# changlin31/AutoProg

Measured on AMD Instinct MI355X. Metric: images/sec/GPU (fwd+bwd) VOLO-D1 224px AutoProg step, higher is better.
Workload: dtype bf16; 1 GPU; BASELINE.json configs[1]: volo_h12_l18 (VOLO-D1) 224px token-label training step; model=volo_h12_l18, global_batch=128, per_gpu_batch=128, res=224, parallelism=dp1, step=fwd+loss+bwd+AdamW+4xEMA, deterministic=False

## Files before the change

autoprog_amd/_lib.py:

```python
import ctypes
import os

import torch
from ctypes import POINTER, Structure, c_char_p, c_float, c_int, c_int64, c_void_p

_HERE = os.path.dirname(os.path.abspath(__file__))
LIB_PATH = os.environ.get("AP_LIB_PATH") or os.path.join(_HERE, "libautoprog_hip.so")


class GemmEpilogue(Structure):
    _fields_ = [("bias", c_void_p), ("gelu", c_int), ("preact_out", c_void_p), ("dgelu_of", c_void_p),
                ("row_scale", c_void_p), ("rows_per_scale", c_int), ("residual", c_void_p), ("ldr", c_int), ("mul_by", c_void_p),
                ("mul_by8", c_void_p), ("q8_out", c_void_p), ("q8_scale", c_void_p), ("q8_amax", c_void_p)]


class MlpFusedArgs(Structure):
    _fields_ = [("x", c_void_p), ("ldx", c_int), ("wa", c_void_p), ("ldwa", c_int), ("wb", c_void_p), ("ldwb", c_int), ("out", c_void_p), ("ldo", c_int),
                ("hidden_out", c_void_p), ("ldh", c_int), ("codes", c_void_p), ("bias1", c_void_p), ("bias2", c_void_p),
                ("row_scale_hidden", c_void_p), ("row_scale_out", c_void_p), ("rows_per_scale", c_int), ("residual", c_void_p), ("ldr", c_int),
                ("m", c_int), ("c", c_int), ("hidden", c_int), ("backward", c_int),
                ("ln_in", c_void_p), ("ld_ln", c_int), ("ln_out", c_void_p), ("ld_lno", c_int), ("ln_gamma", c_void_p), ("ln_beta", c_void_p),
                ("ln_eps", c_float), ("ln_mean", c_void_p), ("ln_rstd", c_void_p)]


# ... 99 lines not shown
_SIGNATURES["ap_conv7_s2d_stat_rows"] = (_I, [_I, _I, _I])
_SIGNATURES["ap_conv7_s2d"] = (_I, [_P, _P, _P, _I, _I, _I, _P, _P])
_SIGNATURES["ap_conv7_s2d_wgrad_workspace"] = (ctypes.c_size_t, [_I, _I, _I])
_SIGNATURES["ap_conv7_s2d_wgrad"] = (_I, [_P, _P, _P, _I, _I, _I, _P, ctypes.c_size_t, _P])
_SIGNATURES["ap_layernorm_bwd_partial"] = (_I, [_P, _P, _P, _P, _P, _P, _P, _L, _I, _P, ctypes.c_size_t, POINTER(c_int), _P])
_SIGNATURES["ap_layernorm_bwd_reduce_batched"] = (_I, [_P, _I, _P])
_SIGNATURES["ap_quantize_fp8"] = (_I, [_P, _P, _L, _P, _P, _P])
_SIGNATURES["ap_quantize_fp8_multi"] = (_I, [_P, _I, _P, _P, _P])
_SIGNATURES["ap_quantize_bf8"] = (_I, [_P, _P, _L, _P, _P, _P, _I, _I, _P, _F, _P, _P])
_SIGNATURES["ap_gemm_tn8_grouped_workspace"] = (ctypes.c_size_t, [_P, _I])
_SIGNATURES["ap_gemm_tn8_acc_grouped"] = (_I, [_P, _I, _P, ctypes.c_size_t, _P])
_SIGNATURES["ap_gemm_tn8_acc_grouped_ln"] = (_I, [_P, _I, _P, _I, _P, ctypes.c_size_t, _P])
_SIGNATURES["ap_debug_poison_lds"] = (_I, [ctypes.c_uint, _P, _P])
_SIGNATURES["ap_conv3x3_c64_bn"] = (_I, [_P, POINTER(BnInput), _P, _P, _I, _I, _I, _P, _P])
_SIGNATURES["ap_conv3x3_c64_wgrad_bn"] = (_I, [_P, POINTER(BnInput), _P, _P, _I, _I, _I, _P, ctypes.c_size_t, _P])
_SIGNATURES["ap_conv3x3_c64_bwd_stats"] = (_I, [_P, _P, _P, _I, _I, _I, _P, POINTER(BnInput), _P, _P])
_SIGNATURES["ap_bn_relu_bwd_act"] = (_I, [_P, _P, _P, _P, _P, _P, _P, _P, _P, _P, _L, _I, _P, ctypes.c_size_t, _P])
_SIGNATURES["ap_bn_relu_bwd_partials"] = (_I, [_P, _P, _P, _P, _P, _P, _P, _I, _P, _P, _P, _L, _I, _P, ctypes.c_size_t, _P])
_SIGNATURES["ap_mhsa_fwd_fp8"] = (_I, [_P, _P, _P, _P, _P, _P, _I, _I, _I, _I, _F, _P, _P])
_SIGNATURES["ap_gemm_nt_fp8"] = (_I, [_P, _I, _P, _I, _P, _I, _I, _I, _I, _P, _P, POINTER(GemmEpilogue), _P])
_SIGNATURES["ap_gemm_nt_patch"] = (_I, [_P, _P, _I, _P, _I, _I, _I, _I, _P, POINTER(PatchMap), _I, _P])
_SIGNATURES["ap_gemm_nt_patch_bn"] = (_I, [_P, POINTER(BnInput), _P, _I, _P, _I, _I, _I, _I, _P, POINTER(PatchMap), _I, _P])
_SIGNATURES["ap_bn_relu_fwd_partials"] = (_I, [_P, _P, _I, _P, _P, _P, _P, _F, _F, _P, _P, _P, _L, _I, _P])
_SIGNATURES["ap_conv3x3_c64_stat_rows"] = (_I, [_I, _I, _I])
_SIGNATURES["ap_conv3x3_c64_pack"] = (_I, [_P, _P, _P, _P])
_SIGNATURES["ap_conv3x3_c64"] = (_I, [_P, _P, _P, _I, _I, _I, _P, _P])
_SIGNATURES["ap_conv3x3_c64_wgrad_workspace"] = (ctypes.c_size_t, [_I, _I, _I])
_SIGNATURES["ap_conv3x3_c64_wgrad"] = (_I, [_P, _P, _P, _I, _I, _I, _P, ctypes.c_size_t, _P])
_SIGNATURES["ap_conv7_s2d_ld"] = (_I, [_P, _P, _P, _I, _I, _I, _I, _P, _P])
_SIGNATURES["ap_conv7_s2d_wgrad_ld"] = (_I, [_P, _P, _I, _P, _I, _I, _I, _P, ctypes.c_size_t, _P])
_SIGNATURES["ap_conv3x3_c128_pack"] = (_I, [_P, _P, _P, _P])
_SIGNATURES["ap_conv3x3_c128_stat_rows"] = (_I, [_I, _I, _I])
_SIGNATURES["ap_conv3x3_c128"] = (_I, [_P, _P, _P, _I, _I, _I, _P, _P])
_SIGNATURES["ap_conv3x3_c128_wgrad_workspace"] = (ctypes.c_size_t, [_I, _I, _I])
_SIGNATURES["ap_conv3x3_c128_wgrad"] = (_I, [_P, _P, _P, _I, _I, _I, _P, ctypes.c_size_t, _P])
_SIGNATURES["ap_sum_reps_acc"] = (_I, [_P, _P, _L, _I, _P])

_SIGNATURES["ap_mlp_fused"] = (_I, [POINTER(MlpFusedArgs), _P])
_SIGNATURES["ap_mlp_fused_infer"] = (_I, [POINTER(MlpFusedArgs), _P])
_SIGNATURES["ap_classify_stats"] = (_I, [_P, _I, _I, _P, _P, _P, _L, _P])
_SIGNATURES["ap_input_prep"] = (_I, [POINTER(InputPrepArgs), _P])
_SIGNATURES["ap_calib_copy"] = (_I, [_P, _P, _L, _P])
_SIGNATURES["ap_calib_mfma"] = (_I, [_P, _P, _I, _P])
_SIGNATURES["ap_grad_health_workspace"] = (ctypes.c_size_t, [_L, _I])
_SIGNATURES["ap_grad_health"] = (_I, [_P, _L, _P, _I, _P, _P, _P, _F, _F, _P, ctypes.c_size_t, _P])
_SIGNATURES["ap_adamw_ema_step_guarded"] = (_I, _SIGNATURES["ap_adamw_ema_step"][1][:-1] + [_P, _P])
_SIGNATURES["ap_adamw_ema_step_ema16"] = (_I, _SIGNATURES["ap_adamw_ema_step"][1][:-1] + [POINTER(c_void_p), _P, _P])
_SIGNATURES["ap_softmax_topk_rows"] = (_I, [_P, _I, _I, _I, _F, _P, _P, _L, _L, _I, _L, _P])
_SIGNATURES["ap_distill_fwd_bwd"] = (_I, [_P, _I, _P, _I, _I, _I, _F, _P, _P, _F, _L, _P])
_SIGNATURES["ap_soft_ce_sparse_gt_fwd_bwd"] = (_I, [_P, _I, _P, _P, _I, _L, _L, _L, _F, _P, _P, _F, _L, _I, _F, _I, _P, _P])
_SIGNATURES["ap_crop_resize_u8"] = (_I, [POINTER(CropResizeArgs), _P])
_SIGNATURES["ap_crop_resample_u8"] = (_I, [POINTER(CropResampleArgs), _P])
_SIGNATURES["ap_randaug_u8"] = (_I, [POINTER(RandAugArgs), _P])

EXPORTED_SYMBOLS = tuple(_SIGNATURES.keys())
EXPECTED_ABI = 7


class AutoProgHipError(RuntimeError):
    pass


def _load():
    if not os.path.isfile(LIB_PATH):
        raise AutoProgHipError(
            "libautoprog_hip.so is missing (%s). Build it with `python -c 'import __graft_entry__ as g; g.build()'` "
            "or `make -C autoprog_amd/csrc`; there is no CPU/PyTorch fallback." % LIB_PATH)
    lib = ctypes.CDLL(LIB_PATH)
    lib.ap_abi_version.restype = ctypes.c_int
    got = lib.ap_abi_version()
    if got != EXPECTED_ABI:
        raise AutoProgHipError("%s has ABI version %d, these bindings were written for %d: rebuild it (make -C autoprog_amd/csrc)"
                               % (LIB_PATH, got, EXPECTED_ABI))
    for name, (res, args) in _SIGNATURES.items():
        fn = getattr(lib, name)
        fn.restype = res
        fn.argtypes = args
    return lib


lib = _load()


def check(code, what):
    if code != 0:
        raise AutoProgHipError("%s failed: %s (code %d)" % (what, lib.ap_error_string(code).decode(), code))
```

autoprog_amd/functional.py:

```python
import math

import os

import torch

from . import ops, wgrad
from ._lib import AutoProgHipError

BF16 = torch.bfloat16


class _WeightBank:

    generation = 0

    @classmethod
    def _key(cls, p):
        return (p.data_ptr(), p._version, cls.generation, tuple(p.shape))

    @staticmethod
    def _flat(p):
        w = p.detach()
        return w.reshape(w.shape[0], -1).contiguous()

# ... 444 lines not shown
    if not keep:
        del n2, m2, r2
    c2 = ops.gemm_nt(a, bank.get(fc2_w), bias=fc2_b, residual=c1)
    if not keep:
        return c2
    return c2, (c0, t0, mc, rc, mt, rt, nc, nt, kv_t, kv_c, q, o, probs, c1, m2, r2, n2, h, a)


class ClassBlockFn(torch.autograd.Function):

    @staticmethod
    def forward(ctx, cls, tok, n1w, n1b, kv_w, kv_b, q_w, q_b, proj_w, proj_b, n2w, n2b, fc1_w, fc1_b, fc2_w, fc2_b, B, N, heads, eps):
        params = (n1w, n1b, kv_w, kv_b, q_w, q_b, proj_w, proj_b, n2w, n2b, fc1_w, fc1_b, fc2_w, fc2_b)
        c2, kept = _class_forward(cls, tok, *params, B, N, heads, eps, keep=True)
        ctx.save_for_backward(*kept, *params)
        ctx.cfg = (B, N, heads, (q_w.shape[0] // heads) ** -0.5)
        ctx.shapes = (cls.shape, tok.shape)
        ctx.set_materialize_grads(False)
        return c2, tok

    @staticmethod
    def backward(ctx, dc2, dtok_pass):
        (c0, t0, mc, rc, mt, rt, nc, nt, kv_t, kv_c, q, o, probs, c1, m2, r2, n2, h, a,
         n1w, n1b, kv_w, kv_b, q_w, q_b, proj_w, proj_b, n2w, n2b, fc1_w, fc1_b, fc2_w, fc2_b) = ctx.saved_tensors
        B, N, heads, scale = ctx.cfg
        params = (n1w, n1b, kv_w, kv_b, q_w, q_b, proj_w, proj_b, n2w, n2b, fc1_w, fc1_b, fc2_w, fc2_b)
        bufs, sunk = wgrad._param_grad_buffers(params)
        (dn1w, dn1b, dkv_w, dkv_b, dq_w, dq_b, dproj_w, dproj_b, dn2w, dn2b, dfc1_w, dfc1_b, dfc2_w, dfc2_b) = bufs
        g = dc2.contiguous() if dc2 is not None else torch.zeros(c0.shape, dtype=BF16, device=c0.device)
        dpass = dtok_pass.reshape(t0.shape).contiguous() if dtok_pass is not None else None
        with wgrad.wgrad_batch() as batch:
            dh = _linear_bwd(g, a, fc2_w, dfc2_w, dfc2_b, **_gelu_bwd_kw(h))
            dn2 = _linear_bwd(dh, n2, fc1_w, dfc1_w, dfc1_b)
            dc1 = ops.layernorm_bwd(dn2, c1, n2w, m2, r2, g, dn2w, dn2b, defer=batch.ln)
            do = _linear_bwd(dc1, o, proj_w, dproj_w, dproj_b)
            dq, dkv_t, dkv_c = ops.class_attn_bwd(q, kv_t, probs, do, B, N + 1, heads, scale, kv_cls=kv_c)
            dnt = _linear_bwd(dkv_t, nt, kv_w, dkv_w, dkv_b)
            dnc_kv = _linear_bwd(dkv_c, nc, kv_w, dkv_w, dkv_b)
            _linear_bwd(dq, nc, q_w, dq_w, dq_b, need_dx=False)
            wq_t = bank.get_t(q_w)
            dnc = ops.gemm_nt(dq, wq_t, n=wq_t.shape[0], k=wq_t.shape[1], residual=dnc_kv)
            dcls = ops.layernorm_bwd(dnc, c0, n1w, mc, rc, dc1, dn1w, dn1b)
            dtok = ops.layernorm_bwd(dnt, t0, n1w, mt, rt, dpass, dn1w, dn1b, defer=batch.ln)
        return (dcls.view(ctx.shapes[0]), dtok.view(ctx.shapes[1]), *wgrad._finish_param_grads(params, bufs, sunk, batch.deferred), None, None, None, None)


def class_block(cls, tok, *args):
    if infer_mode():
        return _class_forward(cls, tok, *args, keep=False), tok
    return ClassBlockFn.apply(cls, tok, *args)


FUSE_POOL_BWD = os.environ.get("AP_FUSE_POOL_BWD", "1") != "0"


def _outlooker_forward(x, n1w, n1b, v_w, v_b, attn_w, attn_b, proj_w, proj_b, n2w, n2b, fc1_w, fc1_b, fc2_w, fc2_b, heads, eps, *, keep):
    B, H, W, C = x.shape
    T = B * H * W
    x2 = x.reshape(T, C).contiguous()
    scale = (C // heads) ** -0.5
    xn1, m1, r1 = ops.layernorm_fwd(x2, n1w, n1b, eps)
    v = ops.gemm_nt(xn1, bank.get(v_w), bias=v_b)
    pooled2 = ops.avgpool2_fwd(xn1.view(B, H, W, C)).view(-1, C)
    if not keep:
        del xn1, m1, r1
    logits = ops.gemm_nt(pooled2, bank.get(attn_w), bias=attn_b)
    if not keep:
        del pooled2
    yo = ops.outlook_fwd(v.view(B, H, W, C), logits, heads, scale)
    if not keep:
        del v, logits
    x1 = ops.gemm_nt(yo.view(T, C), bank.get(proj_w), bias=proj_b, residual=x2)
    if not keep:
        del yo, x2
    xn2, m2, r2 = ops.layernorm_fwd(x1, n2w, n2b, eps)
    a, h = _fc1_fwd(xn2, fc1_w, fc1_b, keep)
    if not keep:
        del xn2, m2, r2
    y = ops.gemm_nt(a, bank.get(fc2_w), bias=fc2_b, residual=x1).view(x.shape)
    if not keep:
        return y
    return y, (x2, m1, r1, xn1, v, pooled2, logits, yo, x1, m2, r2, xn2, h, a)


class OutlookerBlockFn(torch.autograd.Function):

    @staticmethod
    def forward(ctx, x, n1w, n1b, v_w, v_b, attn_w, attn_b, proj_w, proj_b, n2w, n2b, fc1_w, fc1_b, fc2_w, fc2_b,
                heads, eps):
        params = (n1w, n1b, v_w, v_b, attn_w, attn_b, proj_w, proj_b, n2w, n2b, fc1_w, fc1_b, fc2_w, fc2_b)
        y, kept = _outlooker_forward(x, *params, heads, eps, keep=True)
        ctx.save_for_backward(*kept, *params)
        B, H, W, C = x.shape
        ctx.cfg = (B, H, W, C, heads, (C // heads) ** -0.5)
        return y

    @staticmethod
    def backward(ctx, dy):
        (x2, m1, r1, xn1, v, pooled2, logits, yo, x1, m2, r2, xn2, h, a,
         n1w, n1b, v_w, v_b, attn_w, attn_b, proj_w, proj_b, n2w, n2b, fc1_w, fc1_b, fc2_w, fc2_b) = ctx.saved_tensors
        B, H, W, C, heads, scale = ctx.cfg
        T = B * H * W
        params = (n1w, n1b, v_w, v_b, attn_w, attn_b, proj_w, proj_b, n2w, n2b, fc1_w, fc1_b, fc2_w, fc2_b)
        bufs, sunk = wgrad._param_grad_buffers(params)
        (dn1w, dn1b, dv_w, dv_b, dattn_w, dattn_b, dproj_w, dproj_b, dn2w, dn2b, dfc1_w, dfc1_b, dfc2_w, dfc2_b) = bufs
        dy2 = dy.reshape(T, C).contiguous()
        with wgrad.wgrad_batch(sunk, params) as batch:
            dh = _linear_bwd(dy2, a, fc2_w, dfc2_w, dfc2_b, **_gelu_bwd_kw(h))
            dxn2 = _linear_bwd(dh, xn2, fc1_w, dfc1_w, dfc1_b)
            dx1 = ops.layernorm_bwd(dxn2, x1, n2w, m2, r2, dy2, dn2w, dn2b, defer=batch.ln)
            dyo = _linear_bwd(dx1, yo.view(T, C), proj_w, dproj_w, dproj_b)
            dv, dlogits = ops.outlook_bwd(v.view(B, H, W, C), logits, dyo.view(B, H, W, C), heads, scale)
            dpooled = _linear_bwd(dlogits, pooled2, attn_w, dattn_w, dattn_b, n=attn_w.shape[0])
            dxn1 = _linear_bwd(dv.view(T, C), xn1, v_w, dv_w, dv_b)
            dx = ops.layernorm_bwd(dxn1, x2, n1w, m1, r1, dx1, dn1w, dn1b, defer=batch.ln, pool=(dpooled.view(B, (H + 1) // 2, (W + 1) // 2, C), (B, H, W))) if FUSE_POOL_BWD else None
            if dx is None:
                ops.avgpool2_bwd_acc(dpooled.view(B, (H + 1) // 2, (W + 1) // 2, C), dxn1.view(B, H, W, C))
                dx = ops.layernorm_bwd(dxn1, x2, n1w, m1, r1, dx1, dn1w, dn1b, defer=batch.ln)
        return (dx.view(dy.shape), *wgrad._finish_param_grads(params, bufs, sunk, batch.deferred), None, None)


def outlooker_block(x, *args):
    if infer_mode():
        return _outlooker_forward(x, *args, keep=False)
    return OutlookerBlockFn.apply(x, *args)


class LayerNormFn(torch.autograd.Function):
# ... 658 lines not shown
```

autoprog_amd/ops.py:

```python
import ctypes
import math
import os
from collections import namedtuple

import torch

from . import _lib
from ._lib import CropResampleArgs, CropResizeArgs, GemmEpilogue, InputPrepArgs, LnReduce, RandAugArgs, TnProblem, LN_MAX_BATCH, PREP_MAX_BOXES, TN_MAX_GROUP, TN_MAX_GROUP_DET, AutoProgHipError, check, lib

BF16 = torch.bfloat16


_raw_stream = getattr(torch._C, "_cuda_getCurrentRawStream", None)
_cur_device = getattr(torch._C, "_cuda_getDevice", None)


def _stream():
    if _raw_stream is not None and _cur_device is not None:
        return _raw_stream(_cur_device())
    return torch.cuda.current_stream().cuda_stream


def _req_fail(t, dtype, name):
    if not (torch.is_tensor(t) and t.is_cuda):
# ... 521 lines not shown
            if csw is not None:
                _req(csw, BF16, "colsum_weight")
                if csw.numel() < round_up(a.shape[0], 8) or csw.data_ptr() % 16:
                    raise AutoProgHipError("colsum_weight needs ceil(M/8)*8 elements and 16-byte alignment")
            q.colsum_weight = csw.data_ptr() if csw is not None else None
            q.colsum_scale = float(css)
        ptr = ctypes.cast(arr, ctypes.c_void_p)
        ws, ws_bytes = None, 0
        if deterministic:
            ws_bytes = lib.ap_gemm_tn_grouped_workspace(ptr, len(chunk))
            ws = torch.empty(max(ws_bytes // 4, 1), dtype=torch.float32, device=chunk[0].a.device)
        if ln:
            check(lib.ap_gemm_tn_acc_grouped_ln(ptr, len(chunk), ctypes.cast(_ln_reduce_array(ln), ctypes.c_void_p), len(ln), ws.data_ptr() if ws is not None else None,
                                                ws_bytes, _stream()), "ap_gemm_tn_acc_grouped_ln")
            ln = []
        else:
            check(lib.ap_gemm_tn_acc_grouped(ptr, len(chunk), ws.data_ptr() if ws is not None else None, ws_bytes, _stream()), "ap_gemm_tn_acc_grouped")


def colsum_acc(a, out, n=None):
    _req(a, BF16, "a"); _req(out, torch.float32, "out")
    n = out.numel() if n is None else n
    check(lib.ap_colsum_acc(a.data_ptr(), a.shape[1], out.data_ptr(), a.shape[0], n, _stream()), "ap_colsum_acc")
    return out


def outlook_fwd(v, logits, heads, scale):
    _req(v, BF16, "v"); _req(logits, BF16, "logits")
    B, H, W, C = v.shape
    y = torch.empty_like(v)
    check(lib.ap_outlook_fwd(v.data_ptr(), logits.data_ptr(), logits.shape[-1], y.data_ptr(), B, H, W, heads, C // heads,
                             float(scale), _stream()), "ap_outlook_fwd")
    return y


def outlook_bwd(v, logits, dy, heads, scale):
    _req(v, BF16, "v"); _req(logits, BF16, "logits"); _req(dy, BF16, "dy")
    B, H, W, C = v.shape
    dv = torch.empty_like(v)
    dlogits = torch.empty_like(logits)
    check(lib.ap_outlook_bwd(v.data_ptr(), logits.data_ptr(), logits.shape[-1], dy.data_ptr(), dv.data_ptr(), dlogits.data_ptr(),
                             B, H, W, heads, C // heads, float(scale), _stream()), "ap_outlook_bwd")
    return dv, dlogits


def avgpool2_fwd(x):
    _req(x, BF16, "x")
    B, H, W, C = x.shape
    y = torch.empty((B, (H + 1) // 2, (W + 1) // 2, C), dtype=BF16, device=x.device)
    check(lib.ap_avgpool2_fwd(x.data_ptr(), y.data_ptr(), B, H, W, C, _stream()), "ap_avgpool2_fwd")
    return y


def avgpool2_bwd_acc(dpooled, dx):
    _req(dpooled, BF16, "dpooled"); _req(dx, BF16, "dx")
    B, H, W, C = dx.shape
    check(lib.ap_avgpool2_bwd_acc(dpooled.data_ptr(), dx.data_ptr(), B, H, W, C, _stream()), "ap_avgpool2_bwd_acc")
    return dx


def mhsa_emits_fp8(N, hd):
    e = os.environ.get("AP_MHSA_FLASH")
    return (e == "1") if e is not None else (N > 256 or hd == 48)


def mhsa_fwd(qkv, B, N, heads, scale, out_row_scale=None, fp8=None):
    _req(qkv, BF16, "qkv")
    C = qkv.shape[-1] // 3
    out = torch.empty((B * N, C), dtype=BF16, device=qkv.device)
    lse = torch.empty((B, heads, N), dtype=torch.float32, device=qkv.device)
    if fp8 is not None:
        out8 = torch.empty((B * N, C), dtype=torch.uint8, device=qkv.device)
        check(lib.ap_mhsa_fwd_fp8(qkv.data_ptr(), out.data_ptr(), out8.data_ptr(), fp8[0].data_ptr(), fp8[1].data_ptr() if fp8[1] is not None else None,
                                  lse.data_ptr(), B, N, heads, C // heads, float(scale),
                                  out_row_scale.data_ptr() if out_row_scale is not None else None, _stream()), "ap_mhsa_fwd_fp8")
        return out, lse, out8
    check(lib.ap_mhsa_fwd(qkv.data_ptr(), out.data_ptr(), lse.data_ptr(), B, N, heads, C // heads, float(scale),
                          out_row_scale.data_ptr() if out_row_scale is not None else None, _stream()), "ap_mhsa_fwd")
    return out, lse


def mhsa_bwd(qkv, out, dout, lse, B, N, heads, scale):
    _req(qkv, BF16, "qkv"); _req(out, BF16, "out"); _req(dout, BF16, "dout")
    C = qkv.shape[-1] // 3
    dqkv = torch.empty_like(qkv)
    ws_bytes = lib.ap_mhsa_bwd_workspace(B, N, heads, C // heads)
    ws = torch.empty(ws_bytes // 4, dtype=torch.float32, device=qkv.device) if ws_bytes else None
    check(lib.ap_mhsa_bwd(qkv.data_ptr(), out.data_ptr(), dout.data_ptr(), lse.data_ptr(), dqkv.data_ptr(), B, N, heads, C // heads,
                          float(scale), ws.data_ptr() if ws is not None else None, ws_bytes, _stream()), "ap_mhsa_bwd")
    return dqkv


def class_attn_fwd(q, kv, B, N, heads, scale, kv_cls=None):
    _req(q, BF16, "q"); _req(kv, BF16, "kv")
    C = q.shape[-1]
    out = torch.empty((B, C), dtype=BF16, device=q.device)
    probs = torch.empty((B, heads, N), dtype=torch.float32, device=q.device)
    check(lib.ap_class_attn_fwd(q.data_ptr(), kv.data_ptr(), kv_cls.data_ptr() if kv_cls is not None else None, out.data_ptr(), probs.data_ptr(),
                                B, N, heads, C // heads, float(scale), _stream()), "ap_class_attn_fwd")
    return out, probs


def class_attn_bwd(q, kv, probs, dout, B, N, heads, scale, kv_cls=None):
    _req(dout, BF16, "dout")
    dq = torch.empty_like(q)
    dkv = torch.empty_like(kv)
# ... 517 lines not shown
```

include/autoprog_hip.h:

```cpp
#ifndef AUTOPROG_HIP_H
#define AUTOPROG_HIP_H

#include <stddef.h>
#include <stdint.h>

#ifdef __cplusplus
extern "C" {
#endif

typedef void* ap_stream_t;
typedef uint16_t ap_bf16;

enum {
    AP_OK = 0,
    AP_ERR_SHAPE = -1,
    AP_ERR_UNSUPPORTED = -2,
    AP_ERR_LAUNCH = -3,
    AP_ERR_NULL = -4
};

#define AP_MAX_ROWS 0x7fffff00

int ap_abi_version(void);
const char* ap_error_string(int code);
// ... 78 lines not shown
int ap_quantize_fp8(const ap_bf16* x, unsigned char* y, int64_t n, const float* scale, float* amax, ap_stream_t stream);
typedef struct ap_fp8_job { const ap_bf16* x; unsigned char* y; int64_t n; int slot; int pad_; } ap_fp8_job;
int ap_quantize_fp8_multi(const ap_fp8_job* jobs_device, int njobs, const float* scales, float* amax, ap_stream_t stream);

int ap_debug_poison_lds(unsigned pattern, unsigned* scratch2, ap_stream_t stream);
int ap_gemm_nt_fp8(const unsigned char* A, int lda, const unsigned char* B, int ldb, ap_bf16* C, int ldc, int M, int N, int K,
                   const float* dq_a, const float* dq_b, const struct ap_gemm_epilogue* epi, ap_stream_t stream);
int ap_gemm_tn_acc(const ap_bf16* A, int lda, const ap_bf16* B, int ldb, float* C, int ldc,
                   int M, int N1, int N2, float* colsum_A, ap_stream_t stream);
#define AP_TN_MAX_GROUP 32
typedef struct ap_tn_problem {
    const ap_bf16* A; int lda;
    const ap_bf16* B; int ldb;
    float* C; int ldc;
    int M, N1, N2;
    float alpha;
    float* colsum_A;
    const ap_bf16* colsum_weight;
    float colsum_scale;
    const struct ap_patch_map* b_patch;
    const struct ap_bn_input* b_bn;
} ap_tn_problem;
size_t ap_gemm_tn_grouped_workspace(const ap_tn_problem* problems, int count);
int ap_gemm_tn_acc_grouped(const ap_tn_problem* problems, int count, void* workspace, size_t ws_bytes, ap_stream_t stream);
int ap_gemm_tn_acc_grouped_ln(const ap_tn_problem* problems, int count, const ap_ln_reduce* ln_items, int ln_count,
                              void* workspace, size_t ws_bytes, ap_stream_t stream);
#define AP_BF8_COLSUM_SPLITS 64
int ap_quantize_bf8(const ap_bf16* g, unsigned char* y, int64_t n, const float* scale, float* amax, float* colsum, int rows, int cols,
                    const ap_bf16* colsum_weight, float colsum_scale, float* colsum_ws, ap_stream_t stream);
#define AP_FP8_E4M3 0
#define AP_FP8_E5M2 1
typedef struct ap_tn8_problem {
    const unsigned char* A; int lda;
    const unsigned char* B; int ldb;
    float* C; int ldc;
    int M, N1, N2;
    int a_fmt;
    float alpha;
    const float* dq_a; const float* dq_b;
} ap_tn8_problem;
size_t ap_gemm_tn8_grouped_workspace(const ap_tn8_problem* problems, int count);
int ap_gemm_tn8_acc_grouped(const ap_tn8_problem* problems, int count, void* workspace, size_t ws_bytes, ap_stream_t stream);
int ap_gemm_tn8_acc_grouped_ln(const ap_tn8_problem* problems, int count, const ap_ln_reduce* ln_items, int ln_count,
                               void* workspace, size_t ws_bytes, ap_stream_t stream);
int ap_colsum_acc(const ap_bf16* A, int lda, float* out, int M, int N, ap_stream_t stream);

int ap_outlook_fwd(const ap_bf16* v, const ap_bf16* logits, int ldl, ap_bf16* y,
                   int B, int H, int W, int heads, int hd, float scale, ap_stream_t stream);
int ap_outlook_bwd(const ap_bf16* v, const ap_bf16* logits, int ldl, const ap_bf16* dy,
                   ap_bf16* dv, ap_bf16* dlogits, int B, int H, int W, int heads, int hd,
                   float scale, ap_stream_t stream);
int ap_avgpool2_fwd(const ap_bf16* x, ap_bf16* y, int B, int H, int W, int C, ap_stream_t stream);
int ap_avgpool2_bwd_acc(const ap_bf16* dpooled, ap_bf16* dx, int B, int H, int W, int C, ap_stream_t stream);

int ap_mhsa_fwd(const ap_bf16* qkv, ap_bf16* out, float* lse, int B, int N, int heads, int hd,
                float scale, const float* out_row_scale, ap_stream_t stream);
int ap_mhsa_fwd_fp8(const ap_bf16* qkv, ap_bf16* out, unsigned char* out8, const float* q_scale, float* q_amax, float* lse, int B, int N,
                    int heads, int hd, float scale, const float* out_row_scale, ap_stream_t stream);
size_t ap_mhsa_bwd_workspace(int B, int N, int heads, int hd);
int ap_mhsa_bwd(const ap_bf16* qkv, const ap_bf16* out, const ap_bf16* dout, const float* lse,
                ap_bf16* dqkv, int B, int N, int heads, int hd, float scale,
                void* workspace, size_t ws_bytes, ap_stream_t stream);

int ap_class_attn_fwd(const ap_bf16* q, const ap_bf16* kv, const ap_bf16* kv_cls , ap_bf16* out, float* probs,
                      int B, int N, int heads, int hd, float scale, ap_stream_t stream);
int ap_class_attn_bwd(const ap_bf16* q, const ap_bf16* kv, const ap_bf16* kv_cls , const float* probs, const ap_bf16* dout,
                      ap_bf16* dq, ap_bf16* dkv, ap_bf16* dkv_cls , int B, int N, int heads, int hd, float scale,
                      ap_stream_t stream);

int ap_mix_token_swap(const ap_bf16* x, ap_bf16* y, int B, int H, int W, int C,
                      int r0, int r1, int c0, int c1, ap_stream_t stream);
int ap_mix_token_swap_dev(const ap_bf16* x, ap_bf16* y, int B, int H, int W, int C, const int* box_dev, int scale, ap_stream_t stream);

int ap_classify_stats(const ap_bf16* logits, int ld, int n_classes, const int64_t* labels, float* loss, int* rank, int64_t rows,
                      ap_stream_t stream);
int ap_softmax_topk_rows(const ap_bf16* logits, int ld, int C, int K, float inv_temp, int* idx, float* val, int64_t o_sb, int64_t o_sn,
                         int rows_per_batch, int64_t M, ap_stream_t stream);
int ap_distill_fwd_bwd(const ap_bf16* student, int ld_s, const ap_bf16* teacher, int ld_t, int C, int mode, float inv_temp,
                       float* row_loss, ap_bf16* dstudent, float grad_scale, int64_t M, ap_stream_t stream);
int ap_soft_ce_fwd_bwd(const ap_bf16* logits, int ldx, const float* target, int64_t t_sb,
                       int64_t t_sc, int64_t t_sn, int rows_per_batch, float* row_loss,
                       ap_bf16* dlogits, float grad_scale, int64_t M, int C,
                       float mix_lam, int mix_batches, ap_stream_t stream);
int ap_soft_ce_sparse_fwd_bwd(const ap_bf16* logits, int ldx, const int* idx, const float* val, int K, int64_t p_sb, int64_t p_sn,
                              int rows_per_batch, float smoothing, float* row_loss, ap_bf16* dlogits, float grad_scale,
                              int64_t M, int C, float mix_lam, int mix_batches, ap_stream_t stream);
int ap_soft_ce_fwd_bwd_dev(const ap_bf16* logits, int ldx, const float* target, int64_t t_sb, int64_t t_sc, int64_t t_sn, int rows_per_batch,
                           float* row_loss, ap_bf16* dlogits, float grad_scale, int64_t M, int C, float mix_lam, int mix_batches,
                           const float* mix_lam_dev, ap_stream_t stream);
int ap_soft_ce_sparse_fwd_bwd_dev(const ap_bf16* logits, int ldx, const int* idx, const float* val, int K, int64_t p_sb, int64_t p_sn,
                                  int rows_per_batch, float smoothing, float* row_loss, ap_bf16* dlogits, float grad_scale, int64_t M, int C,
                                  float mix_lam, int mix_batches, const float* mix_lam_dev, ap_stream_t stream);
int ap_soft_ce_sparse_gt_fwd_bwd(const ap_bf16* logits, int ldx, const int* idx, const float* val, int K, int64_t p_sb, int64_t p_s0, int64_t p_s1,
                                 float smoothing, float* row_loss, ap_bf16* dlogits, float grad_scale, int64_t B, int C, float mix_lam,
                                 int mix_batches, const float* mix_lam_dev, ap_stream_t stream);
int ap_loss_combine(const float* a, int64_t na, float wa, const float* b, int64_t nb, float wb, float* out, ap_stream_t stream);

int ap_row_scale(const ap_bf16* x, const float* scale, ap_bf16* y, int64_t M, int C,
                 int rows_per_scale, ap_stream_t stream);
int ap_add_bcast(const ap_bf16* a, const ap_bf16* b, ap_bf16* y, int64_t n, int64_t b_elems, ap_stream_t stream);
#define AP_SUM_REPS_MAX (16 * 65535)
int ap_sum_reps_acc(const ap_bf16* x, float* out, int64_t n, int reps, ap_stream_t stream);
int ap_resample_grid(const float* in, int hi, int wi, const float* wy, const float* wx, float* out, int ho, int wo, int C, int accumulate,
                     ap_stream_t stream);

size_t ap_bn_relu_workspace(int64_t T, int C);
// ... 135 lines not shown
```

Measured before the change: 10540 images/sec.

## Fuse outlooker LayerNorm with v-projection/avgpool and proj GEMM with LayerNorm

```diff
diff --git a/autoprog_amd/_lib.py b/autoprog_amd/_lib.py
--- a/autoprog_amd/_lib.py
+++ b/autoprog_amd/_lib.py
@@ -175,6 +175,8 @@
 _SIGNATURES["ap_crop_resize_u8"] = (_I, [POINTER(CropResizeArgs), _P])
 _SIGNATURES["ap_crop_resample_u8"] = (_I, [POINTER(CropResampleArgs), _P])
 _SIGNATURES["ap_randaug_u8"] = (_I, [POINTER(RandAugArgs), _P])
+_SIGNATURES["ap_outlook_ln_v_pool_fwd"] = (_I, [_P, _P, _P, _F, _P, _I, _P, _P, _P, _P, _P, _P, _I, _I, _I, _I, _P])
+_SIGNATURES["ap_outlook_proj_ln_fwd"] = (_I, [_P, _P, _I, _P, _P, _P, _P, _F, _P, _P, _P, _P, _L, _I, _P])
 
 EXPORTED_SYMBOLS = tuple(_SIGNATURES.keys())
 EXPECTED_ABI = 7
diff --git a/autoprog_amd/csrc/gemm_rr.h b/autoprog_amd/csrc/gemm_rr.h
--- /dev/null
+++ b/autoprog_amd/csrc/gemm_rr.h
@@ -0,0 +1,223 @@
+#pragma once
+#include "gemm_ws.h"
+
+#define RR_LDS_GB (2 * WS_K * (int)sizeof(float))
+#define RR_LDS_BYTES (3 * WS_LDS_A + RR_LDS_GB)
+
+struct RrArgs {
+    const bf16_t* X;
+    const bf16_t* W; int ldb;
+    const float* bias;
+    const float* gamma; const float* beta; float eps;
+    bf16_t* xn; float* mean; float* rstd;
+    bf16_t* out;
+    const bf16_t* res;
+    bf16_t* pooled;
+    int M;
+    int R;
+    int Wd;
+    int n_items, per_xcd;
+};
+
+__device__ __forceinline__ void rr_ln(const u32x4* rx, int l, const float* Gb, float eps, float& mu, float& rs, u32x4* ob) {
+    const float invC = 1.0f / (float)WS_K;
+    float v[3][8];
+    float s = 0.f;
+#pragma unroll
+    for (int i = 0; i < 3; ++i) {
+        unpack8(rx[i], v[i]);
+#pragma unroll
+        for (int k = 0; k < 8; ++k) s += v[i][k];
+    }
+    s += __shfl_xor(s, 4, 64); s += __shfl_xor(s, 2, 64); s += __shfl_xor(s, 1, 64);
+    mu = s * invC;
+    float q = 0.f;
+#pragma unroll
+    for (int i = 0; i < 3; ++i)
+#pragma unroll
+        for (int k = 0; k < 8; ++k) { const float d = v[i][k] - mu; q = __builtin_fmaf(d, d, q); }
+    q += __shfl_xor(q, 4, 64); q += __shfl_xor(q, 2, 64); q += __shfl_xor(q, 1, 64);
+    rs = rsqrtf(__builtin_fmaf(q, invC, eps));
+#pragma unroll
+    for (int i = 0; i < 3; ++i) {
+        const int ch = l + 8 * i;
+        const f32x4 g0 = *reinterpret_cast<const f32x4*>(Gb + 8 * ch), g1 = *reinterpret_cast<const f32x4*>(Gb + 8 * ch + 4);
+        const f32x4 b0 = *reinterpret_cast<const f32x4*>(Gb + WS_K + 8 * ch), b1 = *reinterpret_cast<const f32x4*>(Gb + WS_K + 8 * ch + 4);
+        float o8[8];
+#pragma unroll
+        for (int k = 0; k < 4; ++k) {
+            o8[k] = __builtin_fmaf((v[i][k] - mu) * rs, g0[k], b0[k]);
+            o8[4 + k] = __builtin_fmaf((v[i][4 + k] - mu) * rs, g1[k], b1[k]);
+        }
+        ob[i] = pack8(o8);
+    }
+}
+
+template <int TAIL>
+__global__ void __launch_bounds__(512, 2) k_gemm_rr(RrArgs a) {
+    extern __shared__ __attribute__((aligned(16))) unsigned char rr_smem[];
+    unsigned char* const Al = rr_smem;
+    unsigned char* const St = Al + (TAIL ? WS_LDS_A : 2 * WS_LDS_A);
+    float* const Gb = reinterpret_cast<float*>(rr_smem + 3 * WS_LDS_A);
+    const int tid = threadIdx.x, lane = tid & 63, fr = lane & 15, g = lane >> 4;
+    const int wave = __builtin_amdgcn_readfirstlane(tid >> 6);
+    const int grp = wave >> 2, wn = wave & 3, ltid = tid & 255;
+    const int rr = ltid >> 3, l = ltid & 7;
+    unsigned char* const Sg = St + grp * (TAIL ? WS_LDS_A : WS_LDS_A / 2);
+#define RR_BAR() asm volatile("s_waitcnt lgkmcnt(0)\n\ts_barrier" ::: "memory")
+    const int xcd = blockIdx.x & 7, idx = blockIdx.x >> 3;
+    int item = xcd * a.per_xcd + idx;
+    if (idx >= a.per_xcd || item >= a.n_items) return;
+    const int step = gridDim.x;
+
+    u32x4 wfr[3][WS_K / 32];
+#pragma unroll
+    for (int nt = 0; nt < 3; ++nt)
+#pragma unroll
+        for (int ks = 0; ks < WS_K / 32; ++ks) wfr[nt][ks] = ld16(a.W + (int64_t)(48 * wn + 16 * nt + fr) * a.ldb + (4 * ks + g) * 8);
+    for (int id = tid; id < 2 * WS_K; id += 512) Gb[id] = id < WS_K ? a.gamma[id] : a.beta[id - WS_K];
+    const bool has_bias = a.bias != nullptr;
+    float bias[3][4];
+#pragma unroll
+    for (int nt = 0; nt < 3; ++nt)
+#pragma unroll
+        for (int r = 0; r < 4; ++r) bias[nt][r] = has_bias ? a.bias[48 * wn + 16 * nt + 4 * g + r] : 0.f;
+
+    auto row_of = [&](int it, bool& ok) -> int64_t {
+        const int tr = 32 * grp + rr;
+        const int64_t m = (int64_t)it * a.R + tr;
+        int64_t last = (int64_t)it * a.R + a.R - 1;
+        if (last > (int64_t)a.M - 1) last = (int64_t)a.M - 1;
+        ok = tr < a.R && m <= last;
+        return ok ? m : last;
+    };
+    u32x4 xreg[3], rreg[3];
+    auto request = [&](int it) {
+        bool ok; const int64_t m = row_of(it, ok);
+#pragma unroll
+        for (int i = 0; i < 3; ++i) xreg[i] = ld16(a.X + m * WS_K + (l + 8 * i) * 8);
+    };
+    auto request_res = [&](int it) {
+        if constexpr (TAIL) {
+            bool ok; const int64_t m = row_of(it, ok);
+#pragma unroll
+            for (int i = 0; i < 3; ++i) rreg[i] = ld16(a.res + m * WS_K + (l + 8 * i) * 8);
+        }
+    };
+    auto ln_stage = [&](int it, int par) {
+        bool ok; const int64_t m = row_of(it, ok);
+        float mu, rs; u32x4 ob[3];
+        rr_ln(xreg, l, Gb, a.eps, mu, rs, ob);
+        unsigned char* const Ag = Al + par * WS_LDS_A + grp * (WS_LDS_A / 2);
+#pragma unroll
+        for (int i = 0; i < 3; ++i) st16(Ag + ws_off(rr, l + 8 * i), ob[i]);
+        if (ok && a.xn) {
+#pragma unroll
+            for (int i = 0; i < 3; ++i) st16_nt(a.xn + m * WS_K + (l + 8 * i) * 8, ob[i]);
+            if (l == 0) { a.mean[m] = mu; a.rstd[m] = rs; }
+        }
+    };
+
+    __syncthreads();
+    request(item);
+    if constexpr (TAIL) {
+#pragma unroll
+        for (int i = 0; i < 3; ++i) st16(Al + grp * (WS_LDS_A / 2) + ws_off(rr, l + 8 * i), xreg[i]);
+    } else ln_stage(item, 0);
+    request(item + step < a.n_items ? item + step : item);
+    request_res(item);
+    __syncthreads();
+    if (grp == 1) RR_BAR();
+    int par = 0;
+    while (item < a.n_items) {
+        unsigned char* const Ag = Al + (TAIL ? 0 : par * WS_LDS_A) + grp * (WS_LDS_A / 2);
+        RR_BAR();
+        const int next = item + step, next2 = next + step;
+        f32x4 acc[2][3];
+#pragma unroll
+        for (int mt = 0; mt < 2; ++mt)
+#pragma unroll
+            for (int nt = 0; nt < 3; ++nt) acc[mt][nt] = (f32x4){0.f, 0.f, 0.f, 0.f};
+#pragma unroll
+        for (int ks = 0; ks < WS_K / 32; ++ks) {
+            u32x4 af[2];
+#pragma unroll
+            for (int mt = 0; mt < 2; ++mt) af[mt] = ld16(Ag + ws_off(16 * mt + fr, 4 * ks + g));
+#pragma unroll
+            for (int mt = 0; mt < 2; ++mt)
+#pragma unroll
+                for (int nt = 0; nt < 3; ++nt)
+                    acc[mt][nt] = __builtin_amdgcn_mfma_f32_16x16x32_bf16(as_bf16x8(wfr[nt][ks]), as_bf16x8(af[mt]), acc[mt][nt], 0, 0, 0);
+        }
+#pragma unroll
+        for (int mt = 0; mt < 2; ++mt)
+#pragma unroll
+            for (int nt = 0; nt < 3; ++nt) {
+                const int r = 16 * mt + fr, n = 48 * wn + 16 * nt + 4 * g;
+                f32x4 c = acc[mt][nt];
+                if (has_bias) { c[0] += bias[nt][0]; c[1] += bias[nt][1]; c[2] += bias[nt][2]; c[3] += bias[nt][3]; }
+                if constexpr (TAIL) *reinterpret_cast<f32x4*>(Sg + ws_off32(r, n >> 2)) = c;
+                else {
+                    u32x2 pk;
+                    pk[0] = pack_bf2(c[0], c[1]); pk[1] = pack_bf2(c[2], c[3]);
+                    *reinterpret_cast<u32x2*>(Sg + ws_off(r, n >> 3) + ((n & 4) << 1)) = pk;
+                }
+            }
+        RR_BAR();
+        bool ok; const int64_t m = row_of(item, ok);
+        if constexpr (TAIL) {
+#pragma unroll
+            for (int i = 0; i < 3; ++i) st16(Ag + ws_off(rr, l + 8 * i), xreg[i]);
+            u32x4 xb[3];
+#pragma unroll
+            for (int i = 0; i < 3; ++i) {
+                const int p = l + 8 * i;
+                const f32x4 f0 = *reinterpret_cast<const f32x4*>(Sg + ws_off32(rr, 2 * p)), f1 = *reinterpret_cast<const f32x4*>(Sg + ws_off32(rr, 2 * p + 1));
+                float h[8];
+                unpack8(rreg[i], h);
+                float o8[8];
+#pragma unroll
+                for (int k = 0; k < 4; ++k) { o8[k] = f0[k] + h[k]; o8[4 + k] = f1[k] + h[4 + k]; }
+                xb[i] = pack8(o8);
+            }
+            float mu, rs; u32x4 ob[3];
+            rr_ln(xb, l, Gb, a.eps, mu, rs, ob);
+            if (ok) {
+#pragma unroll
+                for (int i = 0; i < 3; ++i) st16_nt(a.out + m * WS_K + (l + 8 * i) * 8, xb[i]);
+#pragma unroll
+                for (int i = 0; i < 3; ++i) st16_nt(a.xn + m * WS_K + (l + 8 * i) * 8, ob[i]);
+                if (l == 0) { a.mean[m] = mu; a.rstd[m] = rs; }
+            }
+        } else {
+            if (next < a.n_items) ln_stage(next, par ^ 1);
+            if (ok) {
+#pragma unroll
+                for (int i = 0; i < 3; ++i) st16_nt(a.out + m * WS_K + (l + 8 * i) * 8, ld16(Sg + ws_off(rr, l + 8 * i)));
+            }
+            const int W2 = a.Wd >> 1;
+            if (tid < W2 * 24) {
+                const int j = tid / 24, c = tid - j * 24;
+                const unsigned char* const At = Al + par * WS_LDS_A;
+                float pa[8] = {0.f, 0.f, 0.f, 0.f, 0.f, 0.f, 0.f, 0.f};
+#pragma unroll
+                for (int d = 0; d < 4; ++d) {
+                    const int tr = (d >> 1) * a.Wd + 2 * j + (d & 1);
+                    float f[8];
+                    unpack8(ld16(At + (tr >> 5) * (WS_LDS_A / 2) + ws_off(tr & 31, c)), f);
+#pragma unroll
+                    for (int k = 0; k < 8; ++k) pa[k] += f[k];
+                }
+#pragma unroll
+                for (int k = 0; k < 8; ++k) pa[k] *= 0.25f;
+                st16(a.pooled + ((int64_t)item * W2 + j) * WS_K + c * 8, pack8(pa));
+            }
+        }
+        request(next2 < a.n_items ? next2 : item);
+        request_res(next < a.n_items ? next : item);
+        item = next;
+        par ^= 1;
+    }
+    if (grp == 0) RR_BAR();
+#undef RR_BAR
+}
diff --git a/autoprog_amd/csrc/gemm_rr.hip b/autoprog_amd/csrc/gemm_rr.hip
--- /dev/null
+++ b/autoprog_amd/csrc/gemm_rr.hip
@@ -0,0 +1,53 @@
+#include "gemm_rr.h"
+#include <cstdlib>
+
+static int rr_grid(int n_items, int* per_xcd) {
+    int cap = ap_cu_count() & ~7;
+    if (const char* e = getenv("AP_OUTLOOK_LN_GRID")) { const int v = atoi(e); if (v >= 1 && v <= 4096) cap = v; }
+    if (cap < 1) cap = 8;
+    int grid = n_items < cap ? n_items : cap;
+    if (grid >= 8) { *per_xcd = grid / 8; grid = 8 * *per_xcd; } else *per_xcd = 1;
+    return grid;
+}
+
+static bool rr_aligned(const void* p) { return (reinterpret_cast<uintptr_t>(p) & 15) == 0; }
+
+extern "C" {
+
+int ap_outlook_ln_v_pool_fwd(const ap_bf16* x, const float* gamma, const float* beta, float eps, const ap_bf16* wv, int ldw, const float* bv,
+                             ap_bf16* xn, float* mean, float* rstd, ap_bf16* v, ap_bf16* pooled, int B, int H, int W, int C, ap_stream_t stream) {
+    if (!x || !gamma || !beta || !wv || !v || !pooled) return AP_ERR_NULL;
+    if ((xn != nullptr) != (mean != nullptr) || (xn != nullptr) != (rstd != nullptr)) return AP_ERR_NULL;
+    if (B <= 0 || H <= 0 || W <= 0 || C <= 0) return AP_ERR_SHAPE;
+    if (C != WS_K || (H & 1) || (W & 1) || 2 * W > WS_BM || ldw < WS_K || (ldw & 7)) return AP_ERR_UNSUPPORTED;
+    if ((int64_t)B * H * W > AP_MAX_ROWS) return AP_ERR_UNSUPPORTED;
+    if (!rr_aligned(x) || (reinterpret_cast<uintptr_t>(wv) & 3) || !rr_aligned(v) || !rr_aligned(pooled) || !rr_aligned(xn)) return AP_ERR_UNSUPPORTED;
+    RrArgs a;
+    a.X = x; a.W = wv; a.ldb = ldw; a.bias = bv; a.gamma = gamma; a.beta = beta; a.eps = eps;
+    a.xn = xn; a.mean = mean; a.rstd = rstd; a.out = v; a.res = nullptr; a.pooled = pooled;
+    a.M = B * H * W; a.R = 2 * W; a.Wd = W; a.n_items = B * (H / 2);
+    const int grid = rr_grid(a.n_items, &a.per_xcd);
+    (void)hipGetLastError();
+    if (const int rc = ap_allow_lds<k_gemm_rr<0>>(RR_LDS_BYTES); rc != AP_OK) return rc;
+    hipLaunchKernelGGL(k_gemm_rr<0>, dim3(grid), dim3(512), RR_LDS_BYTES, (hipStream_t)stream, a);
+    return ap_check_launch();
+}
+
+int ap_outlook_proj_ln_fwd(const ap_bf16* yo, const ap_bf16* wp, int ldw, const float* bp, const ap_bf16* residual, const float* gamma, const float* beta,
+                           float eps, ap_bf16* x1, ap_bf16* xn, float* mean, float* rstd, int64_t rows, int C, ap_stream_t stream) {
+    if (!yo || !wp || !residual || !gamma || !beta || !x1 || !xn || !mean || !rstd) return AP_ERR_NULL;
+    if (rows <= 0 || C <= 0) return AP_ERR_SHAPE;
+    if (C != WS_K || ldw < WS_K || (ldw & 7) || rows > AP_MAX_ROWS) return AP_ERR_UNSUPPORTED;
+    if (!rr_aligned(yo) || (reinterpret_cast<uintptr_t>(wp) & 3) || !rr_aligned(residual) || !rr_aligned(x1) || !rr_aligned(xn)) return AP_ERR_UNSUPPORTED;
+    RrArgs a;
+    a.X = yo; a.W = wp; a.ldb = ldw; a.bias = bp; a.gamma = gamma; a.beta = beta; a.eps = eps;
+    a.xn = xn; a.mean = mean; a.rstd = rstd; a.out = x1; a.res = residual; a.pooled = nullptr;
+    a.M = (int)rows; a.R = WS_BM; a.Wd = 0; a.n_items = (int)((rows + WS_BM - 1) / WS_BM);
+    const int grid = rr_grid(a.n_items, &a.per_xcd);
+    (void)hipGetLastError();
+    if (const int rc = ap_allow_lds<k_gemm_rr<1>>(RR_LDS_BYTES); rc != AP_OK) return rc;
+    hipLaunchKernelGGL(k_gemm_rr<1>, dim3(grid), dim3(512), RR_LDS_BYTES, (hipStream_t)stream, a);
+    return ap_check_launch();
+}
+
+}
diff --git a/autoprog_amd/functional.py b/autoprog_amd/functional.py
--- a/autoprog_amd/functional.py
+++ b/autoprog_amd/functional.py
@@ -520,6 +520,7 @@
 
 
 FUSE_POOL_BWD = os.environ.get("AP_FUSE_POOL_BWD", "1") != "0"
+FUSE_OUTLOOK_LN = os.environ.get("AP_OUTLOOK_FUSE_LN", "1") != "0"
 
 
 def _outlooker_forward(x, n1w, n1b, v_w, v_b, attn_w, attn_b, proj_w, proj_b, n2w, n2b, fc1_w, fc1_b, fc2_w, fc2_b, heads, eps, *, keep):
@@ -527,9 +528,14 @@
     T = B * H * W
     x2 = x.reshape(T, C).contiguous()
     scale = (C // heads) ** -0.5
-    xn1, m1, r1 = ops.layernorm_fwd(x2, n1w, n1b, eps)
-    v = ops.gemm_nt(xn1, bank.get(v_w), bias=v_b)
-    pooled2 = ops.avgpool2_fwd(xn1.view(B, H, W, C)).view(-1, C)
+    fuse_ln = FUSE_OUTLOOK_LN and T > 256
+    front = ops.outlook_ln_v_pool_fwd(x2.view(B, H, W, C), n1w, n1b, eps, bank.get(v_w), v_b, keep=keep) if fuse_ln else None
+    if front is not None:
+        xn1, m1, r1, v, pooled2 = front
+    else:
+        xn1, m1, r1 = ops.layernorm_fwd(x2, n1w, n1b, eps)
+        v = ops.gemm_nt(xn1, bank.get(v_w), bias=v_b)
+        pooled2 = ops.avgpool2_fwd(xn1.view(B, H, W, C)).view(-1, C)
     if not keep:
         del xn1, m1, r1
     logits = ops.gemm_nt(pooled2, bank.get(attn_w), bias=attn_b)
@@ -538,10 +544,15 @@
     yo = ops.outlook_fwd(v.view(B, H, W, C), logits, heads, scale)
     if not keep:
         del v, logits
-    x1 = ops.gemm_nt(yo.view(T, C), bank.get(proj_w), bias=proj_b, residual=x2)
+    tail = ops.outlook_proj_ln_fwd(yo.view(T, C), bank.get(proj_w), proj_b, x2, n2w, n2b, eps) if fuse_ln else None
+    if tail is not None:
+        x1, xn2, m2, r2 = tail
+    else:
+        x1 = ops.gemm_nt(yo.view(T, C), bank.get(proj_w), bias=proj_b, residual=x2)
     if not keep:
         del yo, x2
-    xn2, m2, r2 = ops.layernorm_fwd(x1, n2w, n2b, eps)
+    if tail is None:
+        xn2, m2, r2 = ops.layernorm_fwd(x1, n2w, n2b, eps)
     a, h = _fc1_fwd(xn2, fc1_w, fc1_b, keep)
     if not keep:
         del xn2, m2, r2
diff --git a/autoprog_amd/ops.py b/autoprog_amd/ops.py
--- a/autoprog_amd/ops.py
+++ b/autoprog_amd/ops.py
@@ -597,6 +597,52 @@
     return y
 
 
+def outlook_ln_v_pool_fwd(x, gamma, beta, eps, wv, bv, keep=True, out=None):
+    _req(x, BF16, "x"); _req(gamma, torch.float32, "gamma"); _req(beta, torch.float32, "beta"); _req(wv, BF16, "wv")
+    B, H, W, C = x.shape
+    if wv.shape[0] != C:
+        return None
+    if out is not None:
+        xn, mean, rstd, v, pooled = out
+    else:
+        xn = torch.empty((B * H * W, C), dtype=BF16, device=x.device) if keep else None
+        mean = torch.empty(B * H * W, dtype=torch.float32, device=x.device) if keep else None
+        rstd = torch.empty(B * H * W, dtype=torch.float32, device=x.device) if keep else None
+        v = torch.empty((B * H * W, C), dtype=BF16, device=x.device)
+        pooled = torch.empty((B * ((H + 1) // 2) * ((W + 1) // 2), C), dtype=BF16, device=x.device)
+    ptr = lambda t: t.data_ptr() if t is not None else None
+    rc = lib.ap_outlook_ln_v_pool_fwd(x.data_ptr(), gamma.data_ptr(), beta.data_ptr(), float(eps), wv.data_ptr(), wv.shape[1], ptr(bv),
+                                      ptr(xn), ptr(mean), ptr(rstd), v.data_ptr(), pooled.data_ptr(), B, H, W, C, _stream())
+    if rc == -2:
+        return None
+    check(rc, "ap_outlook_ln_v_pool_fwd")
+    return xn, mean, rstd, v, pooled
+
+
+def outlook_proj_ln_fwd(yo, wp, bp, residual, gamma, beta, eps, out=None):
+    _req(yo, BF16, "yo"); _req(wp, BF16, "wp"); _req(residual, BF16, "residual"); _req(gamma, torch.float32, "gamma"); _req(beta, torch.float32, "beta")
+    C = yo.shape[-1]
+    rows = yo.numel() // C
+    if residual.numel() != yo.numel():
+        raise AutoProgHipError("outlook_proj_ln_fwd: the residual has the product's shape")
+    if wp.shape[0] != C:
+        return None
+    if out is not None:
+        x1, xn, mean, rstd = out
+    else:
+        x1 = torch.empty((rows, C), dtype=BF16, device=yo.device)
+        xn = torch.empty((rows, C), dtype=BF16, device=yo.device)
+        mean = torch.empty(rows, dtype=torch.float32, device=yo.device)
+        rstd = torch.empty(rows, dtype=torch.float32, device=yo.device)
+    rc = lib.ap_outlook_proj_ln_fwd(yo.data_ptr(), wp.data_ptr(), wp.shape[1], bp.data_ptr() if bp is not None else None, residual.data_ptr(),
+                                    gamma.data_ptr(), beta.data_ptr(), float(eps), x1.data_ptr(), xn.data_ptr(), mean.data_ptr(), rstd.data_ptr(),
+                                    rows, C, _stream())
+    if rc == -2:
+        return None
+    check(rc, "ap_outlook_proj_ln_fwd")
+    return x1, xn, mean, rstd
+
+
 def avgpool2_bwd_acc(dpooled, dx):
     _req(dpooled, BF16, "dpooled"); _req(dx, BF16, "dx")
     B, H, W, C = dx.shape
diff --git a/include/autoprog_hip.h b/include/autoprog_hip.h
--- a/include/autoprog_hip.h
+++ b/include/autoprog_hip.h
@@ -154,6 +154,11 @@
                    float scale, ap_stream_t stream);
 int ap_avgpool2_fwd(const ap_bf16* x, ap_bf16* y, int B, int H, int W, int C, ap_stream_t stream);
 int ap_avgpool2_bwd_acc(const ap_bf16* dpooled, ap_bf16* dx, int B, int H, int W, int C, ap_stream_t stream);
+int ap_outlook_ln_v_pool_fwd(const ap_bf16* x, const float* gamma, const float* beta, float eps, const ap_bf16* wv, int ldw, const float* bv,
+                             ap_bf16* xn, float* mean, float* rstd, ap_bf16* v, ap_bf16* pooled, int B, int H, int W, int C, ap_stream_t stream);
+int ap_outlook_proj_ln_fwd(const ap_bf16* yo, const ap_bf16* wp, int ldw, const float* bp, const ap_bf16* residual, const float* gamma,
+                           const float* beta, float eps, ap_bf16* x1, ap_bf16* xn, float* mean, float* rstd, int64_t rows, int C,
+                           ap_stream_t stream);
 
 int ap_mhsa_fwd(const ap_bf16* qkv, ap_bf16* out, float* lse, int B, int N, int heads, int hd,
                 float scale, const float* out_row_scale, ap_stream_t stream);
```

Result: no change. 10620 images/sec (median of 6 runs) (+0.8%).
